# ChuckDanz/DCLIP

Hardware: AMD Instinct MI355X
Metric: distill-step images/sec at ViT-B/32 bs=256 (higher is better)
Workload: dtype f32

## Files before the change

### dclip_amd/_lib.py

```python
from __future__ import annotations

import ctypes as C
import os

_HERE = os.path.dirname(os.path.abspath(__file__))
LIB_PATH = os.environ.get("DCLIP_LIB_PATH") or os.path.join(_HERE, "libdclip_hip.so")

P = C.c_void_p
I = C.c_int
F = C.c_float
Z = C.c_size_t
L = C.c_int64

SIGNATURES = {
    "dclip_abi_version": (I, []),
    "dclip_last_error": (C.c_char_p, []),
    "dclip_last_launch": (C.c_char_p, []),
    "dclip_first_launch": (C.c_char_p, []),
    "dclip_gemm_f32_workspace": (Z, [I, I, I, I, I]),
    "dclip_gemm_f32_plan": (I, [I, I, I, I, I, C.POINTER(C.c_int)]),
    "dclip_gemm_f32": (I, [P, P, P, P, P, P, I, I, I, I, I, I, I, I, F, I, P, Z, P]),
    "dclip_colsum_f32_workspace": (Z, [I, I]),
    "dclip_colsum_f32": (I, [P, P, I, I, I, I, P, Z, P]),
    "dclip_layernorm_fwd": (I, [P, P, P, P, P, P, I, I, F, P]),
# ... 139 lines not shown
    "dclip_gemm_f16x3_scaled_rows_stats_plan": (I, [I, I, I]),
    "dclip_gemm_f16x3_scaled_rows_stats_dev": (I, [P, P, P, P, I, I, I, I, I, I, I, I, I, I, I, P, P, P, P, P]),
    "dclip_gemm_f16x3_wgrad_tokmajor_plan": (I, [I, I, I]),
    "dclip_gemm_f16x3_wgrad_tokmajor_workspace": (Z, [I, I, I]),
    "dclip_gemm_f16x3_wgrad_tokmajor": (I, [P, P, P, I, I, I, I, I, I, I, I, I, I, P, P, I, P, Z, P]),
    "dclip_split_f32_f16x2": (I, [P, P, I, I, I, I, F, P, P]),
    "dclip_attention_fwd_f16x2": (I, [P, P, I, I, I, I, F, I, I, P]),
    "dclip_attention_varlen_fwd_f16x2": (I, [P, P, P, I, I, I, I, F, I, I, P]),
    "dclip_quick_gelu_f32": (I, [P, P, Z, P]),
    "dclip_layernorm_fwd_f16x2": (I, [P, P, P, P, P, P, P, I, I, F, F, P, P]),
    "dclip_split_f32_f16x2_rows": (I, [P, P, P, I, I, I, P]),
    "dclip_split_f32_f16x2_rows_colstats": (I, [P, P, P, P, P, P, P, I, I, I, P, Z, P]),
    "dclip_split_f32_f16x2_rows_cols_stats": (I, [P, P, P, P, P, P, P, P, P, I, I, I, I, P]),
    "dclip_gemm_f16x3_scaled_split2": (I, [P, P, P, P, I, I, I, I, I, I, I, I, I, I, I, F, F, P]),
    "dclip_gemm_f16x3_scaled_split2_dev": (I, [P, P, P, P, P, P, I, I, I, I, I, I, I, I, I, I, I, P, P, P]),
    "dclip_gemm_f16_wgrad_tokmajor_seg3_plan": (I, [I, I, I]),
    "dclip_gemm_f16_wgrad_tokmajor_seg3": (I, [P, P, P, I, I, I, I, I, I, I, I, I, I, I, I, P, P, I, P, Z, P]),
    "dclip_gemm_f16_ex": (I, [P, P, P, P, P, P, I, I, I, I, I, I, I, I, P]),
    "dclip_gemm_f16_wgrad_tokmajor_plan": (I, [I, I, I]),
    "dclip_gemm_f16_wgrad_tokmajor": (I, [P, P, P, I, I, I, I, I, I, I, P, Z, P]),
    "dclip_gemm_f16_splitk_plan": (I, [I, I, I]),
    "dclip_gemm_f16_splitk_workspace": (Z, [I, I, I]),
    "dclip_gemm_f16_splitk": (I, [P, P, P, I, I, I, I, I, I, I, P, Z, P]),
    "dclip_cast_f32_f16_ieee": (I, [P, P, I, I, I, I, P]),
    "dclip_layernorm_fwd_f16_stats": (I, [P, P, P, P, P, P, I, I, F, P]),
    "dclip_layernorm_bwd_ex_f16": (I, [P, P, P, P, P, P, P, P, P, P, P, I, I, I, P, Z, P]),
    "dclip_transpose_to_f16": (I, [P, I, P, P, I, I, I, I, I, P]),
    "dclip_rowsum_f16": (I, [P, P, I, I, I, P]),
    "dclip_colsum_f16": (I, [P, P, I, I, I, I, P, Z, P]),
    "dclip_mt_weights_f16": (I, [P, I, I, P]),
# ... 42 lines not shown
```

### dclip_amd/csrc/embed.hip

```cpp
#include "common.h"

namespace {

inline int grid_for(size_t work) {
  size_t b = (work + 255) / 256;
  return (int)(b < 1 ? 1 : (b > 4096 ? 4096 : b));
}

__global__ void __launch_bounds__(256) im2col_kernel(const float* __restrict__ pix, float* __restrict__ cols, int B, int C,
                                                     int Himg, int Wimg, int p, int g, size_t total) {
  const int kdim = C * p * p;
  for (size_t i = (size_t)blockIdx.x * blockDim.x + threadIdx.x; i < total; i += (size_t)gridDim.x * blockDim.x) {
    const int k = (int)(i % kdim);
    const size_t row = i / kdim;
    const int gx = (int)(row % g), gy = (int)((row / g) % g), b = (int)(row / ((size_t)g * g));
    const int px = k % p, py = (k / p) % p, c = k / (p * p);
    cols[i] = pix[(((size_t)b * C + c) * Himg + gy * p + py) * Wimg + gx * p + px];
  }
}

typedef unsigned short u16x4_e __attribute__((ext_vector_type(4)));
template <class T16>
__global__ void __launch_bounds__(256) im2col_vec_kernel(const float* __restrict__ pix, void* __restrict__ cols, int B, int C,
                                                         int Himg, int Wimg, int p, int g, int ldc, size_t total4) {
  const int kdim4 = C * p * p / 4, p4 = p / 4;
  for (size_t i = (size_t)blockIdx.x * blockDim.x + threadIdx.x; i < total4; i += (size_t)gridDim.x * blockDim.x) {
    const int k4 = (int)(i % kdim4);
    const size_t row = i / kdim4;
    const int gx = (int)(row % g), gy = (int)((row / g) % g), b = (int)(row / ((size_t)g * g));
    const int px = (k4 % p4) * 4, py = (k4 / p4) % p, c = k4 / (p4 * p);
    const f32x4 v = *reinterpret_cast<const f32x4*>(pix + (((size_t)b * C + c) * Himg + gy * p + py) * Wimg + gx * p + px);
    if constexpr (!__is_same(T16, float)) {
      u16x4_e o;
#pragma unroll
      for (int e = 0; e < 4; ++e) o[e] = T16::bits(v[e]);
      *reinterpret_cast<u16x4_e*>(reinterpret_cast<unsigned short*>(cols) + row * ldc + (size_t)k4 * 4) = o;
    } else {
      *reinterpret_cast<f32x4*>(reinterpret_cast<float*>(cols) + row * ldc + (size_t)k4 * 4) = v;
    }
  }
}

__global__ void __launch_bounds__(256) vision_assemble_fwd_kernel(const float* __restrict__ patch, const float* __restrict__ cls,
                                                                  const float* __restrict__ pos, float* __restrict__ x, int B,
                                                                  int S, int D4, size_t total4) {
  for (size_t i = (size_t)blockIdx.x * blockDim.x + threadIdx.x; i < total4; i += (size_t)gridDim.x * blockDim.x) {
    const int d = (int)(i % D4);
    const size_t tok = i / D4;
    const int s = (int)(tok % S);
    const size_t b = tok / S;
    f32x4 v = (s == 0) ? reinterpret_cast<const f32x4*>(cls)[d]
                       : reinterpret_cast<const f32x4*>(patch)[(b * (S - 1) + (s - 1)) * D4 + d];
    reinterpret_cast<f32x4*>(x)[i] = v + reinterpret_cast<const f32x4*>(pos)[(size_t)s * D4 + d];
  }
// ... 178 lines not shown
  hipLaunchKernelGGL((im2col_vec_kernel<T>), dim3(grid_for(total4)), dim3(256), 0, (hipStream_t)stream, pixels, cols, B, C,
                     Himg, Wimg, patch, g, ldc, total4);
  DCLIP_CHECK_LAUNCH(name);
  return DCLIP_OK;
}
}

DCLIP_API int dclip_im2col_bf16(const float* pixels, void* cols, int B, int C, int Himg, int Wimg, int patch, int ldc,
                                void* stream) {
  return im2col16<Bf16T>("im2col_bf16", pixels, cols, B, C, Himg, Wimg, patch, ldc, stream);
}

DCLIP_API int dclip_im2col_f16(const float* pixels, void* cols, int B, int C, int Himg, int Wimg, int patch, int ldc,
                               void* stream) {
  return im2col16<F16T>("im2col_f16", pixels, cols, B, C, Himg, Wimg, patch, ldc, stream);
}

DCLIP_API int dclip_vision_assemble_fwd(const float* patch, const float* cls, const float* pos, float* x, int B, int S, int D,
                                        void* stream) {
  DCLIP_REQUIRE(patch && cls && pos && x, "vision_assemble_fwd: null pointer");
  DCLIP_REQUIRE(B > 0 && S > 1 && D % 4 == 0, "vision_assemble_fwd: bad shape");
  const size_t total4 = (size_t)B * S * D / 4;
  hipLaunchKernelGGL(vision_assemble_fwd_kernel, dim3(grid_for(total4)), dim3(256), 0, (hipStream_t)stream, patch, cls, pos, x,
                     B, S, D / 4, total4);
  DCLIP_CHECK_LAUNCH("vision_assemble_fwd");
  return DCLIP_OK;
}

DCLIP_API int dclip_vision_assemble_bwd(const float* dx, float* dpatch, int B, int S, int D, void* stream) {
  DCLIP_REQUIRE(dx && dpatch, "vision_assemble_bwd: null pointer");
// ... 109 lines not shown
```

### dclip_amd/csrc/gemm_bf16.hip

```cpp
#include "common.h"
#include <stdlib.h>
#include <type_traits>

namespace {

typedef unsigned short u16x4 __attribute__((ext_vector_type(4)));
typedef unsigned int u32x4 __attribute__((ext_vector_type(4)));
typedef unsigned int u32x2 __attribute__((ext_vector_type(2)));

constexpr int BKH = 64;

struct GemmBf16Params {
  const __bf16* A;
  const __bf16* W;
  void* C;
  const float* bias;
  const float* residual;
  int M, N, K;
  int lda, ldw, ldc;
  int epilogue;
  int out_bf16;
  int tiles_m, tiles_n;
  unsigned short* aux;
  int k_per_split;
// ... 1464 lines not shown
  else if (p.alpha_p)
    hipLaunchKernelGGL((gemm_bf16_pp_kernel<F16T, false, true, false, false, false, true>), grid, block, 0, st, p);
  else
    hipLaunchKernelGGL((gemm_bf16_pp_kernel<F16T, false, false, false, false, false, true>), grid, block, 0, st, p);
  DCLIP_CHECK_LAUNCH_V(name, ".pp3");
  return DCLIP_OK;
}
}

DCLIP_API int dclip_gemm_f16x3_plan(int M, int N, int K) {
  if (M <= 0 || N <= 0 || K <= 0 || K % 32 != 0 || !takes_pp(M, N, 3 * K)) return 0;
  const int tiles_min = getenv("DCLIP_F16X3_MIN") ? atoi(getenv("DCLIP_F16X3_MIN")) : 128;
  return (long)cdiv(M, 256) * cdiv(N, 256) >= tiles_min ? 1 : 0;
}

DCLIP_API int dclip_gemm_f16x3_tile_rows(int M, int N, int K, int rows_form, int stats_form) {
  (void)K, (void)rows_form;
  if (M <= 0 || N <= 0) return 256;
  return f16x3_tile_rows(M, N, !stats_form);
}

DCLIP_API int dclip_gemm_f16x3_scaled(const void* A, const void* W, void* C, const float* bias, const float* residual, int M, int N,
                                      int K, int lda, int ldw, int ldc, int a_hi, int a_lo, int w_hi, int w_lo, int epilogue,
                                      int out_f16, float alpha, void* stream) {
  DCLIP_REQUIRE(!(epilogue & DCLIP_EPI_DGELU), "gemm_f16x3_scaled: DGELU is a training epilogue");
  DCLIP_REQUIRE(alpha == alpha && alpha - alpha == 0.f, "gemm_f16x3_scaled: alpha must be finite");
  return gemm16x3("gemm_f16x3_scaled", A, W, C, bias, residual, M, N, K, lda, ldw, ldc, Segs{a_hi, a_lo, w_hi, w_lo}, epilogue, out_f16,
                  stream, alpha, 0.f, nullptr);
}

// ... 423 lines not shown
```

### dclip_amd/csrc/split16.hip

```cpp
#include "common.h"

namespace {

typedef unsigned short u16x4 __attribute__((ext_vector_type(4)));
typedef unsigned short u16x8 __attribute__((ext_vector_type(8)));
typedef unsigned int u32x4s __attribute__((ext_vector_type(4)));
typedef int i32x4s __attribute__((ext_vector_type(4)));

template <int ORDER>
__global__ void __launch_bounds__(256) split_f16x3_kernel(const float* __restrict__ x, unsigned short* __restrict__ y, int rows,
                                                          int cols, int ldx, int ldy, float scale_v,
                                                          const float* __restrict__ scale_p) {
  const float scale = scale_p ? *scale_p : scale_v;
  const int c8 = cols >> 3;
  const size_t total = (size_t)rows * c8;
  for (size_t i = (size_t)blockIdx.x * blockDim.x + threadIdx.x; i < total; i += (size_t)gridDim.x * blockDim.x) {
    const int c = (int)(i % c8) * 8;
    const size_t r = i / c8;
    const f32x4 a = *reinterpret_cast<const f32x4*>(x + r * ldx + c);
    const f32x4 b = *reinterpret_cast<const f32x4*>(x + r * ldx + c + 4);
    u16x8 hi, lo;
#pragma unroll
    for (int e = 0; e < 4; ++e) {
      unsigned short h0, l0, h1, l1;
// ... 982 lines not shown
DCLIP_API int dclip_split16_plan(void* stats, float* plan, int nlayers, int D, void* stream) {
  DCLIP_REQUIRE(stats && plan && nlayers > 0 && D > 0, "split16_plan: bad arguments");
  hipLaunchKernelGGL(split16_plan_kernel, dim3(cdiv(nlayers, 64)), dim3(64), 0, (hipStream_t)stream, (unsigned*)stats, plan, nlayers,
                     __builtin_sqrt((double)D));
  DCLIP_CHECK_LAUNCH("split16_plan");
  return DCLIP_OK;
}

DCLIP_API int dclip_split16_weights(const void* refs, int nrefs, int tiles, const float* plan, void* stream) {
  DCLIP_REQUIRE(refs && plan && nrefs > 0 && tiles > 0, "split16_weights: bad arguments");
  hipLaunchKernelGGL(split16_weights_kernel, dim3(tiles), dim3(256), 0, (hipStream_t)stream, (const Split16Ref*)refs, nrefs, plan);
  DCLIP_CHECK_LAUNCH("split16_weights");
  return DCLIP_OK;
}

DCLIP_API int dclip_split16_weights_t(const void* refs, int nrefs, int tiles, const float* plan, const void* dst_t, void* stream) {
  DCLIP_REQUIRE(refs && plan && dst_t && nrefs > 0 && tiles > 0, "split16_weights_t: bad arguments");
  hipLaunchKernelGGL(split16_weights_t_kernel, dim3(tiles), dim3(256), 0, (hipStream_t)stream, (const Split16Ref*)refs, nrefs, plan,
                     (unsigned short* const*)dst_t);
  DCLIP_CHECK_LAUNCH_V("split16_weights", ".t");
  return DCLIP_OK;
}
```

### dclip_amd/engine.py

```python
from __future__ import annotations

from dataclasses import dataclass
from typing import Dict, List, Optional

import os

import torch

from . import _lib, ops


@dataclass
class LayerParams:
    ln1_w: torch.Tensor
    ln1_b: torch.Tensor
    qkv_w: torch.Tensor
    qkv_b: torch.Tensor
    out_w: torch.Tensor
    out_b: torch.Tensor
    ln2_w: torch.Tensor
    ln2_b: torch.Tensor
    fc1_w: torch.Tensor
    fc1_b: torch.Tensor
    fc2_w: torch.Tensor
# ... 204 lines not shown
    if need_w and isinstance(x, _Remat):
        x = x.make()
    if need_w and need_b:
        gr[bkey] = _galloc(alloc, bkey, (dy.shape[1],), dev)
        gr[wkey] = ops.gemm(dy, x, ops.LAYOUT_TN, out=_galloc(alloc, wkey, (dy.shape[1], x.shape[1]), dev), a_rowsum=gr[bkey])
    elif need_w:
        gr[wkey] = ops.gemm(dy, x, ops.LAYOUT_TN, out=_galloc(alloc, wkey, (dy.shape[1], x.shape[1]), dev))
    elif need_b:
        gr[bkey] = ops.colsum(dy, out=_galloc(alloc, bkey, (dy.shape[1],), dev))
    return None


def _split_wgrad_taken(need_w: bool, sp: Optional[Split16Layer], x3, out_f: int, in_f: int, tokens: int) -> bool:
    return bool(need_w and sp is not None and x3 is not None and _VSPLIT16_WGRAD and
                ops.gemm_f16_wgrad_tokmajor_seg3_plan(out_f, in_f, tokens) > 0)


def _dystats_regime(tokens: int, D: int, I: int) -> bool:
    return bool(_VSPLIT16_DYSTATS and ops.gemm_f16_rows_stats_plan(tokens, I, 3 * D) > 0)


def _with_stats(want: bool, P: int, cols: int, dev):
    return ops.ColStats(P, cols, dev) if want and _VSPLIT16_DYSTATS and P > 0 else None


def _attention_bwd_stats_form(B: int, S: int, H: int, causal: bool):
    P = ops.attention_bwd_stats_plan(B, S, H)
    if P > 0:
        return "stats", P
    P = ops.attention_bwd_rows_stats_plan(B, S, H) if causal else 0
# ... 185 lines not shown
        raise ValueError(f"pixel_values {tuple(pixel_values.shape)} do not make a {gh}x{gw} grid of {v.patch_size}-px patches")
    return ops.pos_interp_fwd(p.pos, v.grid, gh, gw)


def _grid_pos_grad(dpos_cols: torch.Tensor, p: VisionParams, v, grid, alloc, dev) -> torch.Tensor:
    g, D = v.grid, v.hidden_size
    out = _galloc(alloc, "pos", (1 + g * g, D), dev)
    return ops.pos_interp_bwd(dpos_cols.view(-1, D), g, grid[0], grid[1], out=out.view(1 + g * g, D))


def vision_fwd(p: VisionParams, pixel_values: torch.Tensor, cfg, save: bool, hidden_out: Optional[list] = None, grid=None,
               split16_cache: Optional[dict] = None, split16_out: Optional[list] = None):
    v = cfg
    B = pixel_values.shape[0]
    S, D, H = _grid_seq(v, grid), v.hidden_size, v.num_attention_heads
    if grid is None:
        cols, pos = ops.im2col(pixel_values, v.patch_size), p.pos
    else:
        pos = _grid_front(p, pixel_values, v, grid)
        cols = ops.im2col_rect(pixel_values, v.patch_size)
    patch = ops.gemm(cols, p.patch_w.view(D, -1), ops.LAYOUT_NT)
    emb = ops.vision_assemble_fwd(patch, p.class_embedding, pos, B, S, D)
    del patch
    x, m0, r0 = ops.layernorm_fwd(emb, p.pre_w, p.pre_b, v.layer_norm_eps, save_stats=save)
    if hidden_out is not None:
        hidden_out.append(x)
    saved_layers = []
    prune = hidden_out is None and len(p.layers) > 0
    plan, keep = _train_split16(p.layers, v, save, split16_cache, split16_out, _VSPLIT16)
    act = hidden_act(v)
    for li, lp in enumerate(p.layers):
        sp = plan[li] if plan is not None else None
        if prune and li == len(p.layers) - 1:
            cls_tok, sv = last_layer_fwd_cls(x, lp, B, S, H, v.layer_norm_eps, save, sp, keep, act=act)
            saved_layers.append(sv)
            break
# ... 46 lines not shown
            on_ready({f"layers.{i}.{f}": t for f, t in gr.items()})
    return dx


def _vision_tail_bwd(p: VisionParams, d_out, cls_tok, mp, rp, pooled, needd: Dict[str, bool], grads, alloc, on_ready):
    if needd["proj_w"]:
        grads["proj_w"] = ops.gemm(d_out, pooled, ops.LAYOUT_TN, out=_galloc(alloc, "proj_w", tuple(p.proj_w.shape), d_out.device))
    dpooled = ops.gemm(d_out, p.proj_w, ops.LAYOUT_NN)
    dcls, _ = _ln_bwd(dpooled, cls_tok, p.post_w, mp, rp, None, bool(needd["post_w"] or needd["post_b"]), grads, "post_w", "post_b",
                      alloc)
    if on_ready is not None:
        on_ready({n: grads[n] for n in VisionParams.TAIL if grads[n] is not None})
    return dcls


def _vision_head_bwd(p: VisionParams, dx, emb, m0, r0, cols, B: int, S: int, v, grid, needd: Dict[str, bool], grads, alloc, on_ready,
                     k16=None):
    D, dev = v.hidden_size, dx.device
    demb, _ = _ln_bwd(dx, emb, p.pre_w, m0, r0, None, bool(needd["pre_w"] or needd["pre_b"]), grads, "pre_w", "pre_b", alloc)
    if needd["pos"] or needd["class_embedding"]:
        dpos = ops.colsum(demb.view(B, S * D),
                          out=(_galloc(alloc, "pos", (S * D,), dev) if needd["pos"] and grid is None else None))
        if needd["pos"]:
            grads["pos"] = dpos.view(S, D) if grid is None else _grid_pos_grad(dpos, p, v, grid, alloc, dev)
        if needd["class_embedding"]:
            ce = _galloc(alloc, "class_embedding", (D,), dev)
            ce.copy_(dpos[:D])
            grads["class_embedding"] = ce
    if needd["patch_w"]:
        dpatch = ops.vision_assemble_bwd(demb, B, S, D)
        pw = _galloc(alloc, "patch_w", (D, p.patch_w.numel() // D), dev)
        if cols.dtype != torch.float32:
            got = k16.wgrad_tokmajor(k16.cast(dpatch), cols, out=pw)
            if got is None:
                raise RuntimeError("patch-embedding weight gradient: the token-major 16-bit kernel refused a shape its plan accepted")
            grads["patch_w"] = got.view_as(p.patch_w)
        else:
            grads["patch_w"] = ops.gemm(dpatch, cols, ops.LAYOUT_TN, out=pw).view_as(p.patch_w)
    if on_ready is not None:
        on_ready({n: grads[n] for n in VisionParams.HEAD if grads[n] is not None})


def vision_bwd(p: VisionParams, saved, d_out: torch.Tensor, cfg, need: List[bool], on_ready=None, alloc=None, split16=None):
    v = cfg
    cols, emb, m0, r0, saved_layers, cls_tok, mp, rp, pooled, pruned, grid = saved
    B = cls_tok.shape[0]
    S, D, H = _grid_seq(v, grid), v.hidden_size, v.num_attention_heads
    names = p.names()
    needd = dict(zip(names, need))
    grads: Dict[str, Optional[torch.Tensor]] = {n: None for n in names}
    dcls = _vision_tail_bwd(p, d_out, cls_tok, mp, rp, pooled, needd, grads, alloc, on_ready)
    lowest = _lowest_needed(names, needd, VisionParams.HEAD, VisionParams.TAIL)
    if lowest is None:
        return [grads[n] for n in names]
    dx = None if pruned else ops.scatter_rows(dcls, None, B, S, D)
    dx = _layers_bwd(dx, p.layers, saved_layers, needd, grads, lowest, B * S, B, S, H, False, v.layer_norm_eps, split16,
                     alloc=alloc, on_ready=on_ready, dcls=dcls if pruned else None, act=hidden_act(v))
    if lowest < 0:
        _vision_head_bwd(p, dx, emb, m0, r0, cols, B, S, v, grid, needd, grads, alloc, on_ready)
    return [grads[n] for n in names]




class _Ops16:

    def __init__(self, dtype, gemm, layernorm, attention, attention_row, cast, im2col, im2col_rect, attention_varlen,
                 attention_varlen_row):
        self.dtype, self._gemm, self.layernorm, self.attention = dtype, gemm, layernorm, attention
        self.attention_row, self.cast, self.im2col, self.im2col_rect = attention_row, cast, im2col, im2col_rect
        self.attention_varlen, self.attention_varlen_row = attention_varlen, attention_varlen_row

    def gemm(self, a, w, out16: bool = False, **kw):
        if self.dtype == torch.bfloat16:
# ... 802 lines not shown
    ctx3 = _dense_ctx3(B, S, H, False, True)
    for lp, ent in zip(p.layers[:-1], plan[:-1]):
        x = _frozen_split16_layer(x, lp, ent, pc, eps, ctx3)
    cls_tok = _frozen_split16_last_cls(x, p.layers[-1], plan[-1], eps, lambda qkv: ops.attention_cls_fwd(qkv, B, S, H)[0],
                                       lambda xx: ops.gather_rows(xx, None, B, S, D))
    pooled, _, _ = ops.layernorm_fwd(cls_tok, p.post_w, p.post_b, eps, save_stats=False)
    return ops.gemm(pooled, p.proj_w, ops.LAYOUT_NT)



_VSPLIT16 = os.environ.get("DCLIP_VISION_SPLIT16", "1") != "0"
_VSPLIT16_FC1_EPI = os.environ.get("DCLIP_VISION_SPLIT16_FC1_EPI", "1") != "0"
_VSPLIT16_BWD = os.environ.get("DCLIP_VISION_SPLIT16_BWD", "1") != "0"
_VSPLIT16_WGRAD = os.environ.get("DCLIP_VISION_SPLIT16_WGRAD", "1") != "0"
_VSPLIT16_DYSTATS = os.environ.get("DCLIP_VISION_SPLIT16_DYSTATS", "1") != "0"
_SPLIT16_FUSED = os.environ.get("DCLIP_SPLIT16_FUSED", "1")
_SPLIT16_FUSED_K = _SPLIT16_FUSED not in ("0", "tokmajor")
_SPLIT16_FUSED_TOK = _SPLIT16_FUSED not in ("0", "kmajor")
_SPLIT16_PIECES2 = os.environ.get("DCLIP_SPLIT16_PIECES2", "1") != "0"
_VSPLIT16_DROP32 = os.environ.get("DCLIP_VISION_SPLIT16_DROP32", "0") == "1"
_TSPLIT16_ROWS_STATS = os.environ.get("DCLIP_TEXT_SPLIT16_ROWS_STATS", "1") != "0"
_TSPLIT16_KEY, _TSPLIT16_WHAT = "__tsplit16__", "split-fp16 trainable text tower"


def vision_split16_enabled() -> bool:
    return _VSPLIT16


def split16_plan_host(st: Dict[str, float], D: int) -> Dict[str, object]:
    import math
# ... 74 lines not shown
    if host is None:
        return
    flags = host[:, ops.SPLIT16_PLAN_FLAGS].view(torch.int32)
    if bool(flags.any()):
        _split16_log_once(ent.get("what", "split-fp16 vision tower") + ": a weight statistic is non-finite or an activation bound "
                          "needs a scale below 2^-14 (layer flags " +
                          ", ".join(f"{i}:{int(f)}" for i, f in enumerate(flags.tolist()) if f) +
                          "); the forward stays on the split path with that scale and may lose accuracy (" +
                          ent.get("off", "DCLIP_VISION_SPLIT16=0") + " selects the plain fp32 path)")


def vision_split16_check_flags(cache: Optional[dict]) -> None:
    ent = cache.get("__vsplit16__") if cache else None
    if ent is not None:
        _vision_split16_flags(ent)


def _vision_split16_plan(layers: List[LayerParams], cfg, cache: dict, key: str = "__vsplit16__",
                         what: str = "split-fp16 vision tower", off: str = "DCLIP_VISION_SPLIT16=0"):
    if len(layers) == 0 or cfg.hidden_size % 8 or cfg.intermediate_size % 8:
        return None
    capturing = torch.cuda.is_current_stream_capturing()
    ent = cache.get(key)
    ptrs = tuple(getattr(lp, f).data_ptr() for lp in layers for f in _SPLIT16_WATCHED)
    if ent is None or ent["ptrs"] != ptrs:
        if capturing:
            _split16_log_once(what + ": first use inside a graph capture; this capture takes the plain fp32 path "
                              "(run one eager step first)")
            return None
        if any(not getattr(lp, f).is_contiguous() for lp in layers for f in _SPLIT16_WATCHED):
# ... 296 lines not shown
```

### dclip_amd/ops.py

```python
from __future__ import annotations

from typing import Optional

import torch

from . import _lib

A_KMAJOR, B_KMAJOR = 1, 2
EPI_BIAS, EPI_GELU, EPI_DGELU, EPI_RESIDUAL, EPI_ACCUM, EPI_A_ROWSUM = 1, 2, 4, 8, 16, 32
LAYOUT_NT = A_KMAJOR | B_KMAJOR
LAYOUT_NN = A_KMAJOR
LAYOUT_TN = 0


def _stream():
    return torch.cuda.current_stream().cuda_stream


def _f32(t: torch.Tensor, name: str) -> torch.Tensor:
    if not (t.is_cuda and t.dtype == torch.float32 and t.is_contiguous()):
        raise ValueError(f"{name}: expected a contiguous float32 CUDA tensor, got {t.dtype} {t.device} "
                         f"contiguous={t.is_contiguous()}")
    return t

# ... 1640 lines not shown
        splits = lib.dclip_gemm_f16x3_wgrad_tokmajor_plan(M, N, tokens)
        if splits == 0:
            return None
    if _f32(col_alpha, "col_alpha").numel() != M:
        raise ValueError("gemm_f16x3_wgrad_tokmajor: col_alpha size")
    out = _out_f32(out, (M, N), dy.device, "gemm_f16x3_wgrad_tokmajor")
    nbytes = lib.dclip_gemm_f16x3_wgrad_tokmajor_workspace(M, N, splits)
    ws = _ws.get(nbytes, dy.device)
    _lib.check(lib.dclip_gemm_f16x3_wgrad_tokmajor(dy.data_ptr(), x.data_ptr(), out.data_ptr(), M, N, tokens, dy.shape[1], x.shape[1],
                                                   N, *sg, col_alpha.data_ptr(), act_scale_ptr, splits, _ptr(ws), nbytes, _stream()),
               "gemm_f16x3_wgrad_tokmajor")
    return out



def cast_f16_ieee(x: torch.Tensor, pad_to: int = 8, out: Optional[torch.Tensor] = None) -> torch.Tensor:
    lib = _lib.load()
    _f32(x, "x")
    if x.dim() != 2:
        raise ValueError("cast_f16_ieee: x must be 2-D")
    rows, cols = x.shape
    ld = (cols + pad_to - 1) // pad_to * pad_to
    if out is not None:
        if tuple(_f16(out, "out").shape) != (rows, ld):
            raise ValueError(f"cast_f16_ieee: out shape {tuple(out.shape)} != {(rows, ld)}")
        y = out
    else:
        y = torch.empty((rows, ld), dtype=torch.float16, device=x.device)
    _lib.check(lib.dclip_cast_f32_f16_ieee(x.data_ptr(), y.data_ptr(), rows, cols, cols, ld, _stream()), "cast_f32_f16_ieee")
    return y
# ... 525 lines not shown
```

### include/dclip_hip.h

```cpp
#ifndef DCLIP_HIP_H
#define DCLIP_HIP_H

#include <stddef.h>
#include <stdint.h>

#ifdef __cplusplus
extern "C" {
#endif

#define DCLIP_ABI_VERSION 1

enum {
  DCLIP_OK = 0,
  DCLIP_EINVAL = -1,
  DCLIP_EWORKSPACE = -2,
  DCLIP_ELAUNCH = -3
};

int dclip_abi_version(void);
const char* dclip_last_error(void);
const char* dclip_last_launch(void);
const char* dclip_first_launch(void);

#define DCLIP_A_KMAJOR 1
// ... 289 lines not shown
int dclip_quick_gelu_f32(const float* h, float* g, size_t n, void* stream);
int dclip_layernorm_fwd_f16x2(const float* x, const float* gamma, const float* beta, void* y, float* y32, float* mean, float* rstd,
                              int rows, int D, float eps, float scale, const float* scale_dev, void* stream);
int dclip_split_f32_f16x2_rows(const float* x, void* y, float* row_alpha, int rows, int cols, int ldx, void* stream);
int dclip_split_f32_f16x2_rows_colstats(const float* x, void* y, float* row_alpha, void* yc, int* col_exp, float* col_alpha, float* db,
                                        int rows, int cols, int ldx, void* workspace, size_t workspace_bytes, void* stream);
int dclip_split_f32_f16x2_rows_cols_stats(const float* x, void* y, float* row_alpha, void* yc, int* col_exp, float* col_alpha, float* db,
                                          const void* pmax, const float* psum, int P, int rows, int cols, int ldx, void* stream);
int dclip_gemm_f16x3_scaled_split2(const void* A, const void* W, void* C, const float* bias, int M, int N, int K, int lda, int ldw,
                                   int ldc, int a_hi, int a_lo, int w_hi, int w_lo, int epilogue, float alpha, float out_scale,
                                   void* stream);
int dclip_gemm_f16x3_scaled_split2_dev(const void* A, const void* W, void* C, const float* bias, float* h32, float* g32, int M, int N,
                                       int K, int lda, int ldw, int ldc, int a_hi, int a_lo, int w_hi, int w_lo, int epilogue,
                                       const float* alpha, const float* out_scale, void* stream);

int dclip_attention_fwd_f16x2(const float* qkv, void* y, int B, int S, int H, int causal, float scale, int pieces, int ldy,
                              void* stream);
int dclip_attention_varlen_fwd_f16x2(const float* qkv, const int32_t* cu_seqlens, void* y, int N, int max_S, int H, int causal,
                                     float scale, int pieces, int ldy, void* stream);

int dclip_gemm_f16_ex(const void* A, const void* W, void* C, const float* bias, const float* residual, void* aux, int M,
                      int N, int K, int lda, int ldw, int ldc, int epilogue, int out_f16, void* stream);
int dclip_gemm_f16_wgrad_tokmajor_plan(int M, int N, int K);
int dclip_gemm_f16_wgrad_tokmajor(const void* dY, const void* X, float* C, int M, int N, int K, int lddy, int ldx, int ldc,
                                  int splits, void* workspace, size_t workspace_bytes, void* stream);
int dclip_gemm_f16_splitk_plan(int M, int N, int K);
size_t dclip_gemm_f16_splitk_workspace(int M, int N, int splits);
int dclip_gemm_f16_splitk(const void* A, const void* W, float* C, int M, int N, int K, int lda, int ldw, int ldc, int splits,
                          void* workspace, size_t workspace_bytes, void* stream);
int dclip_cast_f32_f16_ieee(const float* x, void* y, int rows, int cols, int ldx, int ldy, void* stream);
// ... 34 lines not shown
```

Measured before the change: 8193.

## Route patch embedding through split-fp16 GEMM with fused im2col split

Adds a split-fp16 path for the vision patch embedding. A fused im2col kernel emits scaled hi/lo fp16 pieces directly. A front kernel computes the pixel and weight absmax on device to pick power-of-two scales, and the weight split into three fp16 pieces is cached. The patch GEMM then runs on the f16x3 matrix-core path instead of the fp32 GEMM, and can keep the split columns for the backward weight gradient. This costs extra absmax and planning launches and a host pinned-copy of flags, and adds accuracy risk if the scales fall out of range.

```diff
diff --git a/dclip_amd/_lib.py b/dclip_amd/_lib.py
--- a/dclip_amd/_lib.py
+++ b/dclip_amd/_lib.py
@@ -177,6 +177,14 @@
     "dclip_split_f32_f16x2_rows_cols_stats": (I, [P, P, P, P, P, P, P, P, P, I, I, I, I, P]),
     "dclip_gemm_f16x3_scaled_split2": (I, [P, P, P, P, I, I, I, I, I, I, I, I, I, I, I, F, F, P]),
     "dclip_gemm_f16x3_scaled_split2_dev": (I, [P, P, P, P, P, P, I, I, I, I, I, I, I, I, I, I, I, P, P, P]),
+    "dclip_im2col_f16x2": (I, [P, P, I, I, I, I, I, F, P, P]),
+    "dclip_split16_front_rec_floats": (I, []),
+    "dclip_split16_front_wrec_floats": (I, []),
+    "dclip_split16_front_workspace": (Z, []),
+    "dclip_split16_front": (I, [P, Z, P, I, I, P, P, P, P, Z, I, P]),
+    "dclip_split_f32_f16x2_cols_workspace": (Z, [I, I]),
+    "dclip_split_f32_f16x2_cols": (I, [P, P, P, P, I, I, I, P, Z, P]),
+    "dclip_split16_patch_plan": (I, [I, I, I]),
     "dclip_gemm_f16_wgrad_tokmajor_seg3_plan": (I, [I, I, I]),
     "dclip_gemm_f16_wgrad_tokmajor_seg3": (I, [P, P, P, I, I, I, I, I, I, I, I, I, I, I, I, P, P, I, P, Z, P]),
     "dclip_gemm_f16_ex": (I, [P, P, P, P, P, P, I, I, I, I, I, I, I, I, P]),
diff --git a/dclip_amd/csrc/embed.hip b/dclip_amd/csrc/embed.hip
--- a/dclip_amd/csrc/embed.hip
+++ b/dclip_amd/csrc/embed.hip
@@ -38,6 +38,33 @@
     } else {
       *reinterpret_cast<f32x4*>(reinterpret_cast<float*>(cols) + row * ldc + (size_t)k4 * 4) = v;
     }
+  }
+}
+
+typedef unsigned short u16x8_e __attribute__((ext_vector_type(8)));
+__global__ void __launch_bounds__(256) im2col_f16x2_kernel(const float* __restrict__ pix, unsigned short* __restrict__ cols, int B,
+                                                           int C, int Himg, int Wimg, int p, int g, float scale_v,
+                                                           const float* __restrict__ scale_p, size_t total8) {
+  const float scale = scale_p ? *scale_p : scale_v;
+  const int kdim = C * p * p, kdim8 = kdim / 8, p8 = p / 8;
+  for (size_t i = (size_t)blockIdx.x * blockDim.x + threadIdx.x; i < total8; i += (size_t)gridDim.x * blockDim.x) {
+    const int k8 = (int)(i % kdim8);
+    const size_t row = i / kdim8;
+    const int gx = (int)(row % g), gy = (int)((row / g) % g), b = (int)(row / ((size_t)g * g));
+    const int px = (k8 % p8) * 8, py = (k8 / p8) % p, c = k8 / (p8 * p);
+    const float* src = pix + (((size_t)b * C + c) * Himg + gy * p + py) * Wimg + gx * p + px;
+    const f32x4 v0 = *reinterpret_cast<const f32x4*>(src), v1 = *reinterpret_cast<const f32x4*>(src + 4);
+    u16x8_e hi, lo;
+#pragma unroll
+    for (int e = 0; e < 4; ++e) {
+      unsigned short h0, l0, h1, l1;
+      split1(v0[e] * scale, h0, l0);
+      split1(v1[e] * scale, h1, l1);
+      hi[e] = h0, lo[e] = l0, hi[4 + e] = h1, lo[4 + e] = l1;
+    }
+    unsigned short* dst = cols + row * 2 * kdim + (size_t)k8 * 8;
+    *reinterpret_cast<u16x8_e*>(dst) = hi;
+    *reinterpret_cast<u16x8_e*>(dst + kdim) = lo;
   }
 }
 
@@ -246,6 +273,22 @@
 DCLIP_API int dclip_im2col_f16(const float* pixels, void* cols, int B, int C, int Himg, int Wimg, int patch, int ldc,
                                void* stream) {
   return im2col16<F16T>("im2col_f16", pixels, cols, B, C, Himg, Wimg, patch, ldc, stream);
+}
+
+DCLIP_API int dclip_im2col_f16x2(const float* pixels, void* cols, int B, int C, int Himg, int Wimg, int patch, float scale,
+                                 const float* scale_dev, void* stream) {
+  DCLIP_REQUIRE(pixels && cols, "im2col_f16x2: null pointer");
+  DCLIP_REQUIRE(B > 0 && C > 0 && patch > 0 && patch % 8 == 0 && Himg == Wimg && Himg % patch == 0,
+                "im2col_f16x2: bad shape %dx%d patch %d (patch must be a multiple of 8)", Himg, Wimg, patch);
+  DCLIP_REQUIRE(((uintptr_t)pixels | (uintptr_t)cols) % 16 == 0 && (uintptr_t)scale_dev % 4 == 0, "im2col_f16x2: alignment");
+  DCLIP_REQUIRE(scale_dev || (scale > 0.f && scale - scale == 0.f && (__builtin_bit_cast(unsigned int, scale) & 0x007fffffu) == 0),
+                "im2col_f16x2: scale must be a power of two");
+  const int g = Himg / patch;
+  const size_t total8 = (size_t)B * g * g * C * patch * patch / 8;
+  hipLaunchKernelGGL(im2col_f16x2_kernel, dim3(grid_for(total8)), dim3(256), 0, (hipStream_t)stream, pixels, (unsigned short*)cols,
+                     B, C, Himg, Wimg, patch, g, scale_dev ? 1.f : scale, scale_dev, total8);
+  DCLIP_CHECK_LAUNCH("im2col_f16x2");
+  return DCLIP_OK;
 }
 
 DCLIP_API int dclip_vision_assemble_fwd(const float* patch, const float* cls, const float* pos, float* x, int B, int S, int D,
diff --git a/dclip_amd/csrc/gemm_bf16.hip b/dclip_amd/csrc/gemm_bf16.hip
--- a/dclip_amd/csrc/gemm_bf16.hip
+++ b/dclip_amd/csrc/gemm_bf16.hip
@@ -1502,6 +1502,12 @@
   return (long)cdiv(M, 256) * cdiv(N, 256) >= tiles_min ? 1 : 0;
 }
 
+DCLIP_API int dclip_split16_patch_plan(int rows, int D, int K) {
+  if (dclip_gemm_f16x3_plan(rows, D, K) == 0) return 0;
+  const int tiles_min = getenv("DCLIP_PATCH_SPLIT16_MIN") ? atoi(getenv("DCLIP_PATCH_SPLIT16_MIN")) : 128;
+  return (long)cdiv(rows, 256) * cdiv(D, 256) >= tiles_min ? 1 : 0;
+}
+
 DCLIP_API int dclip_gemm_f16x3_tile_rows(int M, int N, int K, int rows_form, int stats_form) {
   (void)K, (void)rows_form;
   if (M <= 0 || N <= 0) return 256;
diff --git a/dclip_amd/csrc/split16.hip b/dclip_amd/csrc/split16.hip
--- a/dclip_amd/csrc/split16.hip
+++ b/dclip_amd/csrc/split16.hip
@@ -1020,6 +1020,204 @@
   return DCLIP_OK;
 }
 
+namespace {
+constexpr int FRONT_REC_FLOATS = 8, FRONT_WREC_FLOATS = 4, FRONT_PIX_BLOCKS = 1024, FRONT_W_BLOCKS = 64;
+
+__global__ void __launch_bounds__(256) front_absmax_kernel(const float* __restrict__ pix, size_t npix, const float* __restrict__ w,
+                                                           size_t nw, unsigned* __restrict__ partial) {
+  __shared__ unsigned sm[4];
+  const bool is_w = blockIdx.x >= FRONT_PIX_BLOCKS;
+  const float* x = is_w ? w : pix;
+  const size_t n = is_w ? nw : npix, n4 = n / 4;
+  const size_t blk = is_w ? blockIdx.x - FRONT_PIX_BLOCKS : blockIdx.x, nblk = is_w ? FRONT_W_BLOCKS : FRONT_PIX_BLOCKS;
+  unsigned m = 0u;
+  for (size_t i = blk * 256 + threadIdx.x; i < n4; i += nblk * 256) {
+    const f32x4 v = reinterpret_cast<const f32x4*>(x)[i];
+#pragma unroll
+    for (int e = 0; e < 4; ++e) {
+      const float f = v[e];
+      const unsigned u = __builtin_bit_cast(unsigned, f) & 0x7fffffffu;
+      m = m > u ? m : u;
+    }
+  }
+  if (blk == 0 && n4 * 4 + threadIdx.x < n) {
+    const unsigned u = __builtin_bit_cast(unsigned, x[n4 * 4 + threadIdx.x]) & 0x7fffffffu;
+    m = m > u ? m : u;
+  }
+  m = wave_umax(m);
+  if ((threadIdx.x & 63) == 0) sm[threadIdx.x >> 6] = m;
+  __syncthreads();
+  if (threadIdx.x == 0) {
+    for (int k = 1; k < 4; ++k) m = m > sm[k] ? m : sm[k];
+    partial[blockIdx.x] = m;
+  }
+}
+
+__device__ __forceinline__ unsigned block_umax(unsigned m, unsigned* sm) {
+  m = wave_umax(m);
+  __syncthreads();
+  if ((threadIdx.x & 63) == 0) sm[threadIdx.x >> 6] = m;
+  __syncthreads();
+  if (threadIdx.x == 0)
+    for (int k = 1; k < 4; ++k) m = m > sm[k] ? m : sm[k];
+  return m;
+}
+
+__global__ void __launch_bounds__(256) front_plan_kernel(const unsigned* __restrict__ partial, int have_w, float* __restrict__ wrec,
+                                                         float* __restrict__ rec) {
+  __shared__ unsigned sm[4];
+  unsigned mp = 0u, mw = 0u;
+  for (int i = threadIdx.x; i < FRONT_PIX_BLOCKS; i += 256) mp = mp > partial[i] ? mp : partial[i];
+  mp = block_umax(mp, sm);
+  if (have_w) {
+    if (threadIdx.x < FRONT_W_BLOCKS) mw = partial[FRONT_PIX_BLOCKS + threadIdx.x];
+    mw = block_umax(mw, sm);
+  }
+  if (threadIdx.x != 0) return;
+  int f;
+  unsigned wflags;
+  float wmax;
+  if (have_w) {
+    wflags = 0u;
+    wmax = __builtin_bit_cast(float, mw);
+    f = weight_exp((double)wmax, wflags);
+    if (f > 127) f = 127, wflags |= 4u;
+    wrec[0] = pow2f(f);
+    wrec[1] = __builtin_bit_cast(float, f);
+    wrec[2] = wmax;
+    wrec[3] = __builtin_bit_cast(float, wflags);
+  } else {
+    f = __builtin_bit_cast(int, wrec[1]);
+    wmax = wrec[2];
+    wflags = __builtin_bit_cast(unsigned, wrec[3]);
+  }
+  unsigned flags = wflags;
+  const float pmax = __builtin_bit_cast(float, mp);
+  int e = act_exp((double)pmax, flags);
+  if (e < -126) e = -126, flags |= 4u;
+  if (-(e + f) > 127 || -(e + f) < -126) flags |= 4u;
+  rec[0] = pow2f(e);
+  rec[1] = pow2f(f);
+  rec[2] = pow2f(-(e + f));
+  rec[3] = __builtin_bit_cast(float, flags);
+  rec[4] = pmax;
+  rec[5] = wmax;
+  rec[6] = __builtin_bit_cast(float, e);
+  rec[7] = __builtin_bit_cast(float, f);
+}
+}
+
+DCLIP_API int dclip_split16_front_rec_floats(void) { return FRONT_REC_FLOATS; }
+DCLIP_API int dclip_split16_front_wrec_floats(void) { return FRONT_WREC_FLOATS; }
+DCLIP_API size_t dclip_split16_front_workspace(void) { return (size_t)(FRONT_PIX_BLOCKS + FRONT_W_BLOCKS) * sizeof(unsigned); }
+
+DCLIP_API int dclip_split16_front(const float* pixels, size_t npix, const float* w, int wrows, int wcols, void* w3, float* wrec,
+                                  float* rec, void* workspace, size_t workspace_bytes, int refresh_w, void* stream) {
+  dclip_note_first_launch("", "");
+  DCLIP_REQUIRE(pixels && npix > 0 && wrec && rec, "split16_front: bad arguments");
+  DCLIP_REQUIRE(!refresh_w || (w && w3 && wrows > 0 && wcols > 0 && wcols % 8 == 0), "split16_front: weight [rows][cols % 8 == 0]");
+  DCLIP_REQUIRE(((uintptr_t)pixels | (uintptr_t)workspace) % 16 == 0 && ((uintptr_t)wrec | (uintptr_t)rec) % 4 == 0 &&
+                    (!refresh_w || ((uintptr_t)w | (uintptr_t)w3) % 16 == 0),
+                "split16_front: alignment");
+  if (!workspace || workspace_bytes < dclip_split16_front_workspace()) {
+    dclip_set_error("split16_front: needs %zu workspace bytes, got %zu", dclip_split16_front_workspace(), workspace_bytes);
+    return DCLIP_EWORKSPACE;
+  }
+  hipStream_t st = (hipStream_t)stream;
+  const size_t nw = refresh_w ? (size_t)wrows * wcols : 0;
+  hipLaunchKernelGGL(front_absmax_kernel, dim3(FRONT_PIX_BLOCKS + (refresh_w ? FRONT_W_BLOCKS : 0)), dim3(256), 0, st, pixels, npix,
+                     refresh_w ? w : nullptr, nw, (unsigned*)workspace);
+  DCLIP_CHECK_LAUNCH_V("split16_front", ".max");
+  dclip_note_first_launch("split16_front", ".max");
+  hipLaunchKernelGGL(front_plan_kernel, dim3(1), dim3(256), 0, st, (const unsigned*)workspace, refresh_w ? 1 : 0, wrec, rec);
+  DCLIP_CHECK_LAUNCH_V("split16_front", ".plan");
+  if (!refresh_w) return DCLIP_OK;
+  return split_launch("split16_front", w, w3, wrows, wcols, wcols, 3 * wcols, 1.f, wrec, 1, stream);
+}
+
+namespace {
+constexpr int COLMAX_MAX_BLOCKS = 1024, COLMAX_ROWS_PER_BLOCK = 8;
+inline int colmax_blocks(int rows) {
+  const int b = cdiv(rows, COLMAX_ROWS_PER_BLOCK);
+  return b < COLMAX_MAX_BLOCKS ? b : COLMAX_MAX_BLOCKS;
+}
+
+__global__ void __launch_bounds__(256) colmax_partial_kernel(const float* __restrict__ x, unsigned* __restrict__ pmax, int rows,
+                                                             int cols, int ldx) {
+  const int c4n = cols >> 2;
+  for (int c4 = threadIdx.x; c4 < c4n; c4 += 256) {
+    unsigned m[4] = {0u, 0u, 0u, 0u};
+    for (int r = blockIdx.x; r < rows; r += gridDim.x) {
+      const f32x4 v = *reinterpret_cast<const f32x4*>(x + (size_t)r * ldx + c4 * 4);
+#pragma unroll
+      for (int e = 0; e < 4; ++e) {
+        const float f = v[e];
+        const unsigned u = __builtin_bit_cast(unsigned, f) & 0x7fffffffu;
+        m[e] = m[e] > u ? m[e] : u;
+      }
+    }
+    *reinterpret_cast<u32x4s*>(pmax + (size_t)blockIdx.x * cols + c4 * 4) = u32x4s{m[0], m[1], m[2], m[3]};
+  }
+}
+
+__global__ void __launch_bounds__(256) colmax_finish_kernel(const unsigned* __restrict__ pmax, int* __restrict__ col_exp,
+                                                            float* __restrict__ col_alpha, int nb, int cols) {
+  __shared__ unsigned smax[FIN_GROUPS][FIN_COLS];
+  const int cl = threadIdx.x % FIN_COLS, g = threadIdx.x / FIN_COLS;
+  const int col = blockIdx.x * FIN_COLS + cl;
+  unsigned m = 0u;
+  if (col < cols) {
+#pragma unroll 4
+    for (int b = g; b < nb; b += FIN_GROUPS) {
+      const unsigned pm = pmax[(size_t)b * cols + col];
+      m = m > pm ? m : pm;
+    }
+  }
+  smax[g][cl] = m;
+  __syncthreads();
+  if (g == 0 && col < cols) {
+    for (int k = 1; k < FIN_GROUPS; ++k) m = m > smax[k][cl] ? m : smax[k][cl];
+    const int e = row_exp(m);
+    col_exp[col] = e;
+    col_alpha[col] = pow2f(-e);
+  }
+}
+}
+
+DCLIP_API size_t dclip_split_f32_f16x2_cols_workspace(int rows, int cols) {
+  if (rows <= 0 || cols <= 0) return 0;
+  return (size_t)colmax_blocks(rows) * cols * sizeof(unsigned);
+}
+
+DCLIP_API int dclip_split_f32_f16x2_cols(const float* x, void* yc, int* col_exp, float* col_alpha, int rows, int cols, int ldx,
+                                         void* workspace, size_t workspace_bytes, void* stream) {
+  const char* name = "split_f32_f16x2_cols";
+  dclip_note_first_launch("", "");
+  DCLIP_REQUIRE(x && yc && col_exp && col_alpha && rows > 0 && cols > 0, "%s: bad arguments", name);
+  DCLIP_REQUIRE(cols % 8 == 0, "%s: cols=%d must be a multiple of 8", name, cols);
+  DCLIP_REQUIRE(ldx >= cols && ldx % 4 == 0, "%s: ldx must be a multiple of 4 and >= cols", name);
+  DCLIP_REQUIRE(((uintptr_t)x | (uintptr_t)yc | (uintptr_t)col_exp | (uintptr_t)workspace) % 16 == 0 && (uintptr_t)col_alpha % 4 == 0,
+                "%s: alignment", name);
+  const size_t need = dclip_split_f32_f16x2_cols_workspace(rows, cols);
+  if (!workspace || workspace_bytes < need) {
+    dclip_set_error("%s: needs %zu workspace bytes, got %zu", name, need, workspace_bytes);
+    return DCLIP_EWORKSPACE;
+  }
+  hipStream_t st = (hipStream_t)stream;
+  const int nb = colmax_blocks(rows);
+  hipLaunchKernelGGL(colmax_partial_kernel, dim3(nb), dim3(256), 0, st, x, (unsigned*)workspace, rows, cols, ldx);
+  DCLIP_CHECK_LAUNCH_V(name, ".max");
+  dclip_note_first_launch(name, ".max");
+  hipLaunchKernelGGL(colmax_finish_kernel, dim3(cdiv(cols, FIN_COLS)), dim3(256), 0, st, (const unsigned*)workspace, col_exp, col_alpha,
+                     nb, cols);
+  DCLIP_CHECK_LAUNCH_V(name, ".finish");
+  const size_t blocks = ((size_t)rows * (cols / 8) + 255) / 256;
+  hipLaunchKernelGGL(split_cols_f16x2_kernel, dim3((unsigned)(blocks > 8192 ? 8192 : blocks)), dim3(256), 0, st, x, (const int*)col_exp,
+                     (unsigned short*)yc, rows, cols, ldx);
+  DCLIP_CHECK_LAUNCH_V(name, ".cols");
+  return DCLIP_OK;
+}
+
 DCLIP_API int dclip_split16_weights_t(const void* refs, int nrefs, int tiles, const float* plan, const void* dst_t, void* stream) {
   DCLIP_REQUIRE(refs && plan && dst_t && nrefs > 0 && tiles > 0, "split16_weights_t: bad arguments");
   hipLaunchKernelGGL(split16_weights_t_kernel, dim3(tiles), dim3(256), 0, (hipStream_t)stream, (const Split16Ref*)refs, nrefs, plan,
diff --git a/dclip_amd/engine.py b/dclip_amd/engine.py
--- a/dclip_amd/engine.py
+++ b/dclip_amd/engine.py
@@ -242,6 +242,24 @@
 def _split_wgrad_taken(need_w: bool, sp: Optional[Split16Layer], x3, out_f: int, in_f: int, tokens: int) -> bool:
     return bool(need_w and sp is not None and x3 is not None and _VSPLIT16_WGRAD and
                 ops.gemm_f16_wgrad_tokmajor_seg3_plan(out_f, in_f, tokens) > 0)
+
+
+def patch_split16_taken(save_with_cache: bool, grid, rows: int, D: int, patch_dim: int, backward: bool = False,
+                        on: Optional[bool] = None, plan=None, wplan=None) -> bool:
+    if on is None:
+        on = _VSPLIT16 and _VSPLIT16_PATCH and (not backward or (_VSPLIT16_BWD and _VSPLIT16_WGRAD))
+    if not (on and save_with_cache and grid is None and rows > 0 and patch_dim % 32 == 0 and rows % 64 == 0):
+        return False
+    if (ops.split16_patch_plan if plan is None else plan)(rows, D, patch_dim) <= 0:
+        return False
+    return not backward or (ops.gemm_f16x3_wgrad_tokmajor_plan if wplan is None else wplan)(D, patch_dim, rows) > 0
+
+
+class _PatchSplit:
+    __slots__ = ("cols16", "rec", "pixels", "patch")
+
+    def __init__(self, cols16, rec, pixels, patch: int):
+        self.cols16, self.rec, self.pixels, self.patch = cols16, rec, pixels, patch
 
 
 def _dystats_regime(tokens: int, D: int, I: int) -> bool:
@@ -457,12 +475,16 @@
     v = cfg
     B = pixel_values.shape[0]
     S, D, H = _grid_seq(v, grid), v.hidden_size, v.num_attention_heads
-    if grid is None:
-        cols, pos = ops.im2col(pixel_values, v.patch_size), p.pos
+    front = _patch_split16_front(p, pixel_values, v, save, grid, split16_cache)
+    if front is not None:
+        cols, patch, pos = *_patch_split16_fwd(p, pixel_values, v, *front), p.pos
     else:
-        pos = _grid_front(p, pixel_values, v, grid)
-        cols = ops.im2col_rect(pixel_values, v.patch_size)
-    patch = ops.gemm(cols, p.patch_w.view(D, -1), ops.LAYOUT_NT)
+        if grid is None:
+            cols, pos = ops.im2col(pixel_values, v.patch_size), p.pos
+        else:
+            pos = _grid_front(p, pixel_values, v, grid)
+            cols = ops.im2col_rect(pixel_values, v.patch_size)
+        patch = ops.gemm(cols, p.patch_w.view(D, -1), ops.LAYOUT_NT)
     emb = ops.vision_assemble_fwd(patch, p.class_embedding, pos, B, S, D)
     del patch
     x, m0, r0 = ops.layernorm_fwd(emb, p.pre_w, p.pre_b, v.layer_norm_eps, save_stats=save)
@@ -539,8 +561,20 @@
     return dcls
 
 
+def _patch_split16_wgrad(ps: _PatchSplit, dpatch: torch.Tensor, pw: torch.Tensor, split16) -> torch.Tensor:
+    D, K = pw.shape
+    if (ps.cols16 is not None and split16 is not None and
+            patch_split16_taken(True, None, dpatch.shape[0], D, K, backward=True) and split16.fresh()):
+        yc, _, col_alpha = ops.split_f16x2_cols(dpatch)
+        got = ops.gemm_f16x3_wgrad_tokmajor(yc, ps.cols16, D, K, col_alpha, ps.rec.data_ptr() + 4 * ops.FRONT_SCALE, out=pw)
+        if got is None:
+            raise RuntimeError("patch-embedding weight gradient: the fused token-major kernel refused a shape its plan accepted")
+        return got
+    return ops.gemm(dpatch, ops.im2col(ps.pixels, ps.patch), ops.LAYOUT_TN, out=pw)
+
+
 def _vision_head_bwd(p: VisionParams, dx, emb, m0, r0, cols, B: int, S: int, v, grid, needd: Dict[str, bool], grads, alloc, on_ready,
-                     k16=None):
+                     k16=None, split16=None):
     D, dev = v.hidden_size, dx.device
     demb, _ = _ln_bwd(dx, emb, p.pre_w, m0, r0, None, bool(needd["pre_w"] or needd["pre_b"]), grads, "pre_w", "pre_b", alloc)
     if needd["pos"] or needd["class_embedding"]:
@@ -555,7 +589,9 @@
     if needd["patch_w"]:
         dpatch = ops.vision_assemble_bwd(demb, B, S, D)
         pw = _galloc(alloc, "patch_w", (D, p.patch_w.numel() // D), dev)
-        if cols.dtype != torch.float32:
+        if isinstance(cols, _PatchSplit):
+            grads["patch_w"] = _patch_split16_wgrad(cols, dpatch, pw, split16).view_as(p.patch_w)
+        elif cols.dtype != torch.float32:
             got = k16.wgrad_tokmajor(k16.cast(dpatch), cols, out=pw)
             if got is None:
                 raise RuntimeError("patch-embedding weight gradient: the token-major 16-bit kernel refused a shape its plan accepted")
@@ -582,7 +618,7 @@
     dx = _layers_bwd(dx, p.layers, saved_layers, needd, grads, lowest, B * S, B, S, H, False, v.layer_norm_eps, split16,
                      alloc=alloc, on_ready=on_ready, dcls=dcls if pruned else None, act=hidden_act(v))
     if lowest < 0:
-        _vision_head_bwd(p, dx, emb, m0, r0, cols, B, S, v, grid, needd, grads, alloc, on_ready)
+        _vision_head_bwd(p, dx, emb, m0, r0, cols, B, S, v, grid, needd, grads, alloc, on_ready, split16=split16)
     return [grads[n] for n in names]
 
 
@@ -1415,6 +1451,7 @@
 _VSPLIT16_BWD = os.environ.get("DCLIP_VISION_SPLIT16_BWD", "1") != "0"
 _VSPLIT16_WGRAD = os.environ.get("DCLIP_VISION_SPLIT16_WGRAD", "1") != "0"
 _VSPLIT16_DYSTATS = os.environ.get("DCLIP_VISION_SPLIT16_DYSTATS", "1") != "0"
+_VSPLIT16_PATCH = os.environ.get("DCLIP_VISION_SPLIT16_PATCH", "1") != "0"
 _SPLIT16_FUSED = os.environ.get("DCLIP_SPLIT16_FUSED", "1")
 _SPLIT16_FUSED_K = _SPLIT16_FUSED not in ("0", "tokmajor")
 _SPLIT16_FUSED_TOK = _SPLIT16_FUSED not in ("0", "kmajor")
@@ -1519,6 +1556,86 @@
     ent = cache.get("__vsplit16__") if cache else None
     if ent is not None:
         _vision_split16_flags(ent)
+    ent = cache.get(_VPATCH16_KEY) if cache else None
+    if ent is not None:
+        _patch_split16_flags(ent)
+
+
+_VPATCH16_KEY = "__vpatch16__"
+
+
+def split16_front_host(max_pixels: float, max_w: float) -> Dict[str, int]:
+    import math
+    flags = 0
+    if math.isfinite(max_w):
+        f = split16_weight_exp(max_w)
+    else:
+        flags, f = flags | 2, 0
+    if f > 127:
+        f, flags = 127, flags | 4
+    e = split16_act_exp(max_pixels)
+    if e is None:
+        if not math.isfinite(max_pixels) or max_pixels < 0.0:
+            flags, e = flags | 2, 0
+        else:
+            flags |= 1
+            m, ex = math.frexp(max_pixels)
+            e = _SPLIT16_TOP - (ex - 1 if m == 0.5 else ex)
+    if e < -126:
+        e, flags = -126, flags | 4
+    if not -126 <= -(e + f) <= 127:
+        flags |= 4
+    return {"e": e, "f": f, "a": max(-126, min(127, -(e + f))), "flags": flags}
+
+
+def _patch_split16_flags(ent: dict) -> None:
+    host = ent["host"]
+    if host is None:
+        return
+    flags = int(host[ops.FRONT_FLAGS:ops.FRONT_FLAGS + 1].view(torch.int32)[0])
+    if flags:
+        _split16_log_once(f"split-fp16 patch embedding: max|pixel_values| or max|patch_w| is non-finite, or the pixels need a scale "
+                          f"below 2^-14 (flags {flags}); the forward stays on the split path with that scale and may lose accuracy "
+                          "(DCLIP_VISION_SPLIT16_PATCH=0 selects the fp32 patch embedding)")
+
+
+def _patch_split16_front(p: "VisionParams", pixel_values: torch.Tensor, v, save: bool, grid, cache: Optional[dict]):
+    D = v.hidden_size
+    K = p.patch_w.numel() // D
+    Bn, _, Hh, Ww = pixel_values.shape
+    if v.patch_size <= 0 or Hh != Ww or Hh % v.patch_size:
+        return None
+    rows = Bn * (Hh // v.patch_size) ** 2
+    if not patch_split16_taken(bool(save and cache is not None), grid, rows, D, K) or hidden_act(v) == GELU_ERF:
+        return None
+    w = p.patch_w.view(D, K)
+    capturing = torch.cuda.is_current_stream_capturing()
+    ent = cache.get(_VPATCH16_KEY)
+    if ent is None or ent["ptr"] != w.data_ptr() or tuple(ent["state"]["w3"].shape) != (D, 3 * K):
+        if capturing:
+            _split16_log_once("split-fp16 patch embedding: first use inside a graph capture; this capture takes the fp32 patch "
+                              "embedding (run one eager step first)")
+            return None
+        ent = {"ptr": w.data_ptr(), "version": None, "state": ops.split16_front_state(w), "host": None}
+        try:
+            ent["host"] = torch.zeros((8,), dtype=torch.float32).pin_memory()
+        except RuntimeError:
+            ent["host"] = None
+        cache[_VPATCH16_KEY] = ent
+    _patch_split16_flags(ent)
+    rec = ops.split16_front(pixel_values, w, ent["state"], capturing or ent["version"] != w._version)
+    ent["version"] = None if capturing else w._version
+    if ent["host"] is not None:
+        ent["host"].copy_(rec, non_blocking=True)
+    return rec, ent["state"]["w3"]
+
+
+def _patch_split16_fwd(p: "VisionParams", pixel_values: torch.Tensor, v, rec: torch.Tensor, w3: torch.Tensor):
+    base = rec.data_ptr()
+    cols16 = ops.im2col_f16x2(pixel_values, v.patch_size, scale_ptr=base + 4 * ops.FRONT_SCALE)
+    patch = ops.gemm_f16x3_dev(cols16, w3, base + 4 * ops.FRONT_ALPHA, pieces=2)
+    keep = patch_split16_taken(True, None, cols16.shape[0], w3.shape[0], w3.shape[1] // 3, backward=True)
+    return _PatchSplit(cols16 if keep else None, rec, pixel_values, v.patch_size), patch
 
 
 def _vision_split16_plan(layers: List[LayerParams], cfg, cache: dict, key: str = "__vsplit16__",
diff --git a/dclip_amd/ops.py b/dclip_amd/ops.py
--- a/dclip_amd/ops.py
+++ b/dclip_amd/ops.py
@@ -1678,6 +1678,67 @@
 
 
 
+FRONT_SCALE, FRONT_WSCALE, FRONT_ALPHA, FRONT_FLAGS, FRONT_PIX_MAX, FRONT_W_MAX, FRONT_E, FRONT_F = range(8)
+
+
+def split16_patch_plan(rows: int, D: int, K: int) -> int:
+    return int(_lib.load().dclip_split16_patch_plan(rows, D, K))
+
+
+def im2col_f16x2(pixels: torch.Tensor, patch: int, scale: float = 1.0, scale_ptr: Optional[int] = None) -> torch.Tensor:
+    lib = _lib.load()
+    _f32(pixels, "pixel_values")
+    B, Cc, Hh, Ww = pixels.shape
+    if patch <= 0 or Hh != Ww or Hh % patch or patch % 8:
+        raise ValueError(f"im2col_f16x2: image {Hh}x{Ww}, patch {patch} (a square image of whole patches, patch % 8 == 0)")
+    g = Hh // patch
+    cols = torch.empty((B * g * g, 2 * Cc * patch * patch), dtype=torch.float16, device=pixels.device)
+    _lib.check(lib.dclip_im2col_f16x2(pixels.data_ptr(), cols.data_ptr(), B, Cc, Hh, Ww, patch, float(scale), scale_ptr, _stream()),
+               "im2col_f16x2")
+    return cols
+
+
+def split16_front_state(w: torch.Tensor) -> dict:
+    lib = _lib.load()
+    _f32(w, "w")
+    if w.dim() != 2 or w.shape[1] % 8:
+        raise ValueError("split16_front_state: w is [D, K] with K % 8 == 0")
+    return {"wrec": torch.zeros((lib.dclip_split16_front_wrec_floats(),), dtype=torch.float32, device=w.device),
+            "w3": torch.empty((w.shape[0], 3 * w.shape[1]), dtype=torch.float16, device=w.device)}
+
+
+def split16_front(pixels: torch.Tensor, w: torch.Tensor, state: dict, refresh_w: bool) -> torch.Tensor:
+    lib = _lib.load()
+    _f32(pixels, "pixel_values"), _f32(w, "w")
+    rec = torch.empty((lib.dclip_split16_front_rec_floats(),), dtype=torch.float32, device=pixels.device)
+    w3 = state["w3"]
+    if tuple(w3.shape) != (w.shape[0], 3 * w.shape[1]):
+        raise ValueError("split16_front: the state was made for another weight shape")
+    nbytes = lib.dclip_split16_front_workspace()
+    ws = _ws.get(nbytes, pixels.device)
+    _lib.check(lib.dclip_split16_front(pixels.data_ptr(), pixels.numel(), w.data_ptr(), w.shape[0], w.shape[1], w3.data_ptr(),
+                                       state["wrec"].data_ptr(), rec.data_ptr(), _ptr(ws), nbytes, int(bool(refresh_w)), _stream()),
+               "split16_front")
+    return rec
+
+
+def split_f16x2_cols(x: torch.Tensor):
+    lib = _lib.load()
+    if x.dtype != torch.float32 or not x.is_cuda or x.dim() != 2 or x.stride(1) != 1:
+        raise ValueError("split_f16x2_cols: x must be a 2-D fp32 device tensor with unit column stride")
+    rows, cols = x.shape
+    dev = x.device
+    yc = torch.empty((rows, 2 * cols), dtype=torch.float16, device=dev)
+    ce = torch.empty((cols,), dtype=torch.int32, device=dev)
+    ca = torch.empty((cols,), dtype=torch.float32, device=dev)
+    nbytes = lib.dclip_split_f32_f16x2_cols_workspace(rows, cols)
+    ws = _ws.get(nbytes, dev)
+    _lib.check(lib.dclip_split_f32_f16x2_cols(x.data_ptr(), yc.data_ptr(), ce.data_ptr(), ca.data_ptr(), rows, cols,
+                                              x.stride(0) if rows > 1 else cols, _ptr(ws), nbytes, _stream()), "split_f32_f16x2_cols")
+    return yc, ce, ca
+
+
+
 def cast_f16_ieee(x: torch.Tensor, pad_to: int = 8, out: Optional[torch.Tensor] = None) -> torch.Tensor:
     lib = _lib.load()
     _f32(x, "x")
diff --git a/include/dclip_hip.h b/include/dclip_hip.h
--- a/include/dclip_hip.h
+++ b/include/dclip_hip.h
@@ -327,6 +327,18 @@
                                        int K, int lda, int ldw, int ldc, int a_hi, int a_lo, int w_hi, int w_lo, int epilogue,
                                        const float* alpha, const float* out_scale, void* stream);
 
+int dclip_im2col_f16x2(const float* pixels, void* cols, int B, int C, int Himg, int Wimg, int patch, float scale,
+                       const float* scale_dev, void* stream);
+int dclip_split16_front_rec_floats(void);
+int dclip_split16_front_wrec_floats(void);
+size_t dclip_split16_front_workspace(void);
+int dclip_split16_front(const float* pixels, size_t npix, const float* w, int wrows, int wcols, void* w3, float* wrec, float* rec,
+                        void* workspace, size_t workspace_bytes, int refresh_w, void* stream);
+size_t dclip_split_f32_f16x2_cols_workspace(int rows, int cols);
+int dclip_split_f32_f16x2_cols(const float* x, void* yc, int* col_exp, float* col_alpha, int rows, int cols, int ldx, void* workspace,
+                               size_t workspace_bytes, void* stream);
+int dclip_split16_patch_plan(int rows, int D, int K);
+
 int dclip_attention_fwd_f16x2(const float* qkv, void* y, int B, int S, int H, int causal, float scale, int pieces, int ldy,
                               void* stream);
 int dclip_attention_varlen_fwd_f16x2(const float* qkv, const int32_t* cu_seqlens, void* y, int N, int max_S, int H, int causal,
```

New measurement: 8352 (median of 6 runs). +1.9%, better.
